# facebookresearch/metamorph

Measured on NVIDIA H100. Metric: interleaved tokens/sec (train step) LLaMA-3-8B+SigLIP seq4096, higher is better.
Workload: dtype bf16

## Files before the change

### metamorph_b200/csrc/gemm_tcgen05.cu

```cuda
#include "wgmma.cuh"
#include <mutex>
#include <stdlib.h>

namespace {

constexpr int BM = 128;
constexpr int BK = 64;
constexpr int kThreads = 384;
constexpr int kStageLd = 68;

enum Epilogue : int {
  EPI_STORE = 0,
  EPI_BIAS = 1,
  EPI_BIAS_GELU_ERF = 2,
  EPI_BIAS_GELU_TANH = 3,
  EPI_RESID = 4,
  EPI_BIAS_RESID = 5,
  EPI_SWIGLU = 6,
  EPI_SWIGLU_BWD = 7,
};

struct EpiParams {
  void* C;
  long long ldc;
  const bf16* bias;
  const bf16* resid;
  long long ldr;
  bf16* aux;
  long long ld_aux;
  int epi;
  int out_f32;
  int accumulate;
  float alpha;
};

template <int BN>
struct Cfg {
  static constexpr int kStages = (BN == 256) ? 3 : 5;
  static constexpr int kABytes = BM * BK * 2;
  static constexpr int kBBytes = BN * BK * 2;
  static constexpr int kStageBytes = kABytes + kBBytes;
  static constexpr int kEpiBytes = 2 * 64 * kStageLd * 4;
  static constexpr int kSmemBytes = kStages * kStageBytes + kEpiBytes + 1024  + 256 ;
  static_assert(kSmemBytes <= 227 * 1024, "shared memory budget of one H100 CTA");
};

__device__ __forceinline__ void epilogue_chunk(const EpiParams& ep, float (&v)[32], int row, bool row_ok,
                                               int col0, int N) {
    const bool full_chunk = (col0 + 32 <= N);

    if (ep.epi == EPI_SWIGLU_BWD) {
      if (row_ok) {
        bf16* gp = ep.aux + (long long)row * ep.ld_aux + 2 * col0;
        bf16* cp = reinterpret_cast<bf16*>(ep.C) + (long long)row * ep.ldc + col0;
#pragma unroll
        for (int blk = 0; blk < 2; ++blk) {
          uint32_t og[8], ou[8], oa[8];
#pragma unroll
          for (int hv = 0; hv < 2; ++hv) {
            const int4 graw = *reinterpret_cast<const int4*>(gp + blk * 32 + hv * 8);
            const int4 uraw = *reinterpret_cast<const int4*>(gp + blk * 32 + 16 + hv * 8);
            const uint32_t ug[4] = {(uint32_t)graw.x, (uint32_t)graw.y, (uint32_t)graw.z, (uint32_t)graw.w};
            const uint32_t uu[4] = {(uint32_t)uraw.x, (uint32_t)uraw.y, (uint32_t)uraw.z, (uint32_t)uraw.w};
#pragma unroll
            for (int j = 0; j < 4; ++j) {
              const float2 g = unpack_bf16x2(ug[j]);
              const float2 u = unpack_bf16x2(uu[j]);
              const float d0 = v[blk * 16 + hv * 8 + 2 * j], d1 = v[blk * 16 + hv * 8 + 2 * j + 1];
              const float s0 = 1.f / (1.f + __expf(-g.x)), s1 = 1.f / (1.f + __expf(-g.y));
              const float a0 = g.x * s0, a1 = g.y * s1;
// ... 102 lines not shown
            f = unpack_bf16x2(old.y); v[j + 2] += f.x; v[j + 3] += f.y;
            f = unpack_bf16x2(old.z); v[j + 4] += f.x; v[j + 5] += f.y;
            f = unpack_bf16x2(old.w); v[j + 6] += f.x; v[j + 7] += f.y;
          }
          int4 o;
          o.x = pack_bf16x2(v[j], v[j + 1]);
          o.y = pack_bf16x2(v[j + 2], v[j + 3]);
          o.z = pack_bf16x2(v[j + 4], v[j + 5]);
          o.w = pack_bf16x2(v[j + 6], v[j + 7]);
          *reinterpret_cast<int4*>(cp + j) = o;
        }
      } else {
        for (int j = 0; j < 32; ++j)
          if (col0 + j < N) {
            float x = v[j];
            if (ep.accumulate) x += __bfloat162float(cp[j]);
            cp[j] = __float2bfloat16(x);
          }
      }
    }
}

template <int BN, int TA, int TB>
__device__ __forceinline__ void wgmma_k16(float (&d)[BN / 2], uint64_t da, uint64_t db, uint32_t acc) {
  if constexpr (BN == 256) wgmma_m64n256_ss<TA, TB>(d, da, db, acc);
  else wgmma_m64n128_ss<TA, TB>(d, da, db, acc);
}

template <int BN, bool A_MN, bool B_MN>
__global__ void __launch_bounds__(kThreads, 1)
gemm_wgmma_kernel(const __grid_constant__ CUtensorMap tmap_a, const __grid_constant__ CUtensorMap tmap_b, int M, int N,
                  int K, int group_m, EpiParams ep) {
  using C = Cfg<BN>;
  extern __shared__ uint8_t smem_raw[];
  const uint32_t smem_base = (smem_u32(smem_raw) + 1023u) & ~1023u;
  const uint32_t epi_base = smem_base + C::kStages * C::kStageBytes;
  const uint32_t bar_base = epi_base + C::kEpiBytes;
  auto full_bar = [&](int s) { return bar_base + 8u * s; };
  auto empty_bar = [&](int s) { return bar_base + 8u * (C::kStages + s); };

  const int wg = threadIdx.x >> 7, lane = threadIdx.x & 31;
  const int num_m = (M + BM - 1) / BM, num_n = (N + BN - 1) / BN;
  const int num_tiles = num_m * num_n;
  const int num_kb = (K + BK - 1) / BK;

  if (threadIdx.x == 0) {
    prefetch_tmap(&tmap_a);
    prefetch_tmap(&tmap_b);
    for (int s = 0; s < C::kStages; ++s) {
      mbar_init(full_bar(s), 1);
      mbar_init(empty_bar(s), 8);
    }
    fence_barrier_init();
  }
  __syncthreads();

  auto tile_coords = [&](int t, int& m_blk, int& n_blk) {
    const int per_group = group_m * num_n;
    const int g = t / per_group;
    const int first_m = g * group_m;
    const int gsz = min(group_m, num_m - first_m);
    const int r = t - g * per_group;
    m_blk = first_m + (r % gsz);
    n_blk = r / gsz;
  };

  if (wg == 0) {
    setmaxnreg_dec<40>();
    if (threadIdx.x == 0) {
      int s = 0;
      uint32_t phase = 0;
      for (int t = blockIdx.x; t < num_tiles; t += gridDim.x) {
        int m_blk, n_blk;
        tile_coords(t, m_blk, n_blk);
        const int m0 = m_blk * BM, n0 = n_blk * BN;
        for (int kb = 0; kb < num_kb; ++kb) {
          mbar_wait(empty_bar(s), phase ^ 1);
          const uint32_t sa = smem_base + s * C::kStageBytes;
          const uint32_t sb = sa + C::kABytes;
          mbar_arrive_expect_tx(full_bar(s), C::kStageBytes);
          const int k0 = kb * BK;
          if constexpr (!A_MN) {
            tma_load_2d(sa, &tmap_a, full_bar(s), k0, m0);
          } else {
#pragma unroll
            for (int j = 0; j < BM / 64; ++j) tma_load_2d(sa + j * (BK * 128), &tmap_a, full_bar(s), m0 + 64 * j, k0);
          }
          if constexpr (!B_MN) {
            tma_load_2d(sb, &tmap_b, full_bar(s), k0, n0);
          } else {
#pragma unroll
            for (int j = 0; j < BN / 64; ++j) tma_load_2d(sb + j * (BK * 128), &tmap_b, full_bar(s), n0 + 64 * j, k0);
          }
          if (++s == C::kStages) { s = 0; phase ^= 1; }
        }
      }
    }
  } else {
    setmaxnreg_inc<232>();
    const int c = wg - 1;
    const int tid = threadIdx.x & 127, warp_in_wg = tid >> 5;
    constexpr uint32_t a_kstep = A_MN ? (16 * 128) : 32, b_kstep = B_MN ? (16 * 128) : 32;
    constexpr uint32_t a_lbo = A_MN ? (BK * 128) : 16, b_lbo = B_MN ? (BK * 128) : 16;
    float* stage = reinterpret_cast<float*>(smem_raw + (epi_base - smem_u32(smem_raw))) + c * 64 * kStageLd;
    const int er = tid & 63, ehalf = tid >> 6;
    int s = 0;
    uint32_t phase = 0;
    float d[BN / 2];
    for (int t = blockIdx.x; t < num_tiles; t += gridDim.x) {
      int m_blk, n_blk;
      tile_coords(t, m_blk, n_blk);
      for (int kb = 0; kb < num_kb; ++kb) {
        mbar_wait(full_bar(s), phase);
        const uint32_t sa = smem_base + s * C::kStageBytes + c * (64 * 128);
        const uint32_t sb = smem_base + s * C::kStageBytes + C::kABytes;
        wgmma_fence();
#pragma unroll
        for (int k = 0; k < BK / 16; ++k)
          wgmma_k16<BN, A_MN, B_MN>(d, wgmma_desc(sa + k * a_kstep, a_lbo), wgmma_desc(sb + k * b_kstep, b_lbo),
                                    (kb | k) != 0 ? 1u : 0u);
        wgmma_commit();
        wgmma_wait<0>();
        __syncwarp();
        if (lane == 0) mbar_arrive(empty_bar(s));
        if (++s == C::kStages) { s = 0; phase ^= 1; }
      }
      const int row = m_blk * BM + c * 64 + er;
      const bool row_ok = row < M;
      const int g = warp_in_wg * 16 + (lane >> 2), q2 = (lane & 3) * 2;
#pragma unroll
      for (int cc = 0; cc < BN / 64; ++cc) {
        const int colc = n_blk * BN + cc * 64;
        if (colc >= N) break;
        asm volatile("bar.sync %0, 128;" ::"r"(1 + c) : "memory");
#pragma unroll
        for (int j = 0; j < 8; ++j) {
          const float* src = d + 4 * (cc * 8 + j);
          *reinterpret_cast<float2*>(stage + g * kStageLd + j * 8 + q2) = make_float2(src[0], src[1]);
          *reinterpret_cast<float2*>(stage + (g + 8) * kStageLd + j * 8 + q2) = make_float2(src[2], src[3]);
        }
        asm volatile("bar.sync %0, 128;" ::"r"(1 + c) : "memory");
        const int col0 = colc + ehalf * 32;
        if (col0 < N) {
          float v[32];
          const float* rp = stage + er * kStageLd + ehalf * 32;
#pragma unroll
          for (int j = 0; j < 32; j += 4) {
            const float4 x = *reinterpret_cast<const float4*>(rp + j);
            v[j] = x.x * ep.alpha; v[j + 1] = x.y * ep.alpha; v[j + 2] = x.z * ep.alpha; v[j + 3] = x.w * ep.alpha;
          }
          epilogue_chunk(ep, v, row, row_ok, col0, N);
        }
      }
    }
  }
}

typedef CUresult (*PFN_encodeTiled)(CUtensorMap*, CUtensorMapDataType, cuuint32_t, void*,
                                    const cuuint64_t*, const cuuint64_t*, const cuuint32_t*,
                                    const cuuint32_t*, CUtensorMapInterleave, CUtensorMapSwizzle,
                                    CUtensorMapL2promotion, CUtensorMapFloatOOBfill);

PFN_encodeTiled get_encode_fn() {
  static PFN_encodeTiled fn = nullptr;
  static std::once_flag once;
  std::call_once(once, [] {
    void* p = nullptr;
    cudaDriverEntryPointQueryResult qres;
    if (cudaGetDriverEntryPoint("cuTensorMapEncodeTiled", &p, cudaEnableDefault, &qres) ==
            cudaSuccess &&
        qres == cudaDriverEntryPointSuccess)
      fn = reinterpret_cast<PFN_encodeTiled>(p);
  });
  return fn;
}

int make_tmap(CUtensorMap* tm, const void* base, long long inner, long long outer, long long ld,
              int box_inner, int box_outer) {
  PFN_encodeTiled enc = get_encode_fn();
  if (!enc) {
    mm_set_error("cuTensorMapEncodeTiled entry point unavailable (no CUDA driver?)");
    return MM_ERR_CUDA;
  }
  cuuint64_t dims[2] = {(cuuint64_t)inner, (cuuint64_t)outer};
// ... 112 lines not shown
```

### metamorph_b200/csrc/attention_bwd_tc.cu

```cuda
#include "attention_tc.cuh"

using namespace mm_attn_tc;

namespace {

constexpr int BW_THREADS = 384;
constexpr int BW_TILE = 32768;
constexpr int BW_SMEM = 6 * BW_TILE + 2048  + 256  + 1024 ;

struct BwdTcParams {
  const float* lse;
  float* lse2;
  float* delta;
  bf16* dq;
  bf16* dk;
  bf16* dv;
  const int* seqlens;
  const int* seg_start;
  const int2* work_q;
  const int2* work_k;
  long long lddq, lddk, lddv;
  int B, T, Tp, Hq, Hkv;
  float scale;
};

__device__ __forceinline__ void store_acc_rows(bf16* dst0, bf16* dst1, bool w0, bool w1, bool ok0, bool ok1,
                                               const float (&a)[64], int q2) {
#pragma unroll
  for (int t = 0; t < 16; ++t) {
    if (w0) *reinterpret_cast<uint32_t*>(dst0 + 8 * t + q2) = ok0 ? pack_bf16x2(a[4 * t], a[4 * t + 1]) : 0u;
    if (w1) *reinterpret_cast<uint32_t*>(dst1 + 8 * t + q2) = ok1 ? pack_bf16x2(a[4 * t + 2], a[4 * t + 3]) : 0u;
  }
}

__global__ void __launch_bounds__(BW_THREADS, 1)
flash_bwd_dq_kernel(const __grid_constant__ CUtensorMap tmap_q, const __grid_constant__ CUtensorMap tmap_k,
                    const __grid_constant__ CUtensorMap tmap_v, const __grid_constant__ CUtensorMap tmap_do,
                    const __grid_constant__ CUtensorMap tmap_o, BwdTcParams p) {
  extern __shared__ uint8_t smem_raw[];
// ... 108 lines not shown
  }
  const int g = ((threadIdx.x & 127) >> 5) * 16 + (lane >> 2), q2 = (lane & 3) * 2;
  int q_idx[2];
  bool q_ok[2];
  float delta[2], lse2[2];
#pragma unroll
  for (int i = 0; i < 2; ++i) {
    const int r = c * 64 + g + 8 * i;
    q_idx[i] = q0 + r;
    q_ok[i] = q_idx[i] < kv_len;
    delta[i] = q_ok[i] ? (sRed[r] + sRed[128 + r]) * p.scale : 0.f;
    lse2[i] = q_ok[i] ? p.lse[((long long)b * p.Hq + h) * p.T + q_idx[i]] * kLog2e : 0.f;
  }
  const float sl2 = p.scale * kLog2e;
  const uint32_t sQc = sQ + (uint32_t)c * 8192u, sdOc = sdO + (uint32_t)c * 8192u;
  float dq[64];
  for (int j = 0; j < n_tiles; ++j) {
    const int bf = j & 1;
    const uint32_t ph = (uint32_t)((j >> 1) & 1);
    mbar_wait(bf ? k_full1 : k_full0, ph);
    mbar_wait(bf ? v_full1 : v_full0, ph);
#pragma unroll 1
    for (int hf = 0; hf < 2; ++hf) {
      float s[32], dp[32];
      wgmma_fence();
#pragma unroll
      for (int k = 0; k < 8; ++k) {
        wgmma_m64n64_ss<0, 0>(s, desc_kmajor(sQc, k), desc_kmajor(sK[bf] + hf * 8192u, k), k != 0 ? 1u : 0u);
        wgmma_m64n64_ss<0, 0>(dp, desc_kmajor(sdOc, k), desc_kmajor(sV[bf] + hf * 8192u, k), k != 0 ? 1u : 0u);
      }
      wgmma_commit();
      wgmma_wait<0>();
      const int k0 = j * 128 + hf * 64;
#pragma unroll
      for (int t = 0; t < 32; ++t) {
        const int i = (t >> 1) & 1;
        const int col = k0 + (t >> 2) * 8 + q2 + (t & 1);
        const bool ok = q_ok[i] && col <= q_idx[i] && col < kv_len;
        const float pv = ok ? fast_exp2(fmaf(s[t], sl2, -lse2[i])) : 0.f;
        s[t] = pv * fmaf(dp[t], p.scale, -delta[i]);
      }
      uint32_t da[4][4];
#pragma unroll
      for (int k = 0; k < 4; ++k) acc_to_a(s, k, da[k]);
      wgmma_fence();
#pragma unroll
      for (int k = 0; k < 4; ++k)
        wgmma_m64n128_rs<1>(dq, da[k], desc_mnmajor(sK[bf], hf * 4 + k), (j | hf | k) != 0 ? 1u : 0u);
      wgmma_commit();
      wgmma_wait<0>();
    }
    consumer_release(bf ? k_empty1 : k_empty0);
    consumer_release(bf ? v_empty1 : v_empty0);
  }
  bf16* d0 = p.dq + (long long)(tok0 + q_idx[0]) * p.lddq + (long long)h * 128;
  bf16* d1 = p.dq + (long long)(tok0 + q_idx[1]) * p.lddq + (long long)h * 128;
  store_acc_rows(d0, d1, q_idx[0] < row_limit, q_idx[1] < row_limit, q_ok[0], q_ok[1], dq, q2);
}

__global__ void __launch_bounds__(BW_THREADS, 1)
flash_bwd_dkv_kernel(const __grid_constant__ CUtensorMap tmap_q, const __grid_constant__ CUtensorMap tmap_k,
                     const __grid_constant__ CUtensorMap tmap_v, const __grid_constant__ CUtensorMap tmap_do,
                     const __grid_constant__ CUtensorMap tmap_stat, BwdTcParams p) {
  extern __shared__ uint8_t smem_raw[];
  const int wg = threadIdx.x >> 7, lane = threadIdx.x & 31;
  const int jt = p.work_k ? 2 * p.work_k[blockIdx.x >> 1].y + (int)(blockIdx.x & 1) : (int)blockIdx.y;
  const int hk = p.work_k ? (int)blockIdx.y : (int)(blockIdx.x % p.Hkv);
  const int b = p.work_k ? p.work_k[blockIdx.x >> 1].x : (int)(blockIdx.x / p.Hkv);
  const int G = p.Hq / p.Hkv;
  const int kv0 = jt * 64;
  const int kv_len = p.seqlens ? min(p.seqlens[b], p.T) : p.T;
  const int tok0 = p.seg_start ? p.seg_start[b] : b * p.T;
  const int row_limit = p.seg_start ? kv_len : p.T;

  if (kv0 >= kv_len) {
    for (int i = threadIdx.x; i < 64 * 16; i += BW_THREADS) {
      const int r = i >> 4, c = (i & 15) * 8;
      if (kv0 + r < row_limit) {
        *reinterpret_cast<int4*>(p.dk + (long long)(tok0 + kv0 + r) * p.lddk + (long long)hk * 128 + c) = make_int4(0, 0, 0, 0);
        *reinterpret_cast<int4*>(p.dv + (long long)(tok0 + kv0 + r) * p.lddv + (long long)hk * 128 + c) = make_int4(0, 0, 0, 0);
      }
    }
    return;
  }
  const int qt_begin = kv0 / 128;
  const int n_qt = (kv_len + 127) / 128 - qt_begin;
  const int n_it = n_qt * G;

  const uint32_t base = (smem_u32(smem_raw) + 1023u) & ~1023u;
  uint8_t* base_ptr = smem_raw + (base - smem_u32(smem_raw));
  const uint32_t sK = base, sV = base + BW_TILE;
  const uint32_t sQ[2] = {base + 2 * BW_TILE, base + 4 * BW_TILE};
  const uint32_t sdO[2] = {base + 3 * BW_TILE, base + 5 * BW_TILE};
  const float* sStat = reinterpret_cast<const float*>(base_ptr + 6 * BW_TILE);
  const uint32_t uStat = base + 6 * BW_TILE;
  const uint32_t bar = base + 6 * BW_TILE + 2048;
  const uint32_t kv_full = bar, qdo_full0 = bar + 8, qdo_full1 = bar + 16, qdo_empty0 = bar + 24, qdo_empty1 = bar + 32;

  if (threadIdx.x == 0) {
    prefetch_tmap(&tmap_q);
    prefetch_tmap(&tmap_k);
    prefetch_tmap(&tmap_v);
    prefetch_tmap(&tmap_do);
    prefetch_tmap(&tmap_stat);
    mbar_init(kv_full, 1);
    mbar_init(qdo_full0, 1);
    mbar_init(qdo_full1, 1);
    mbar_init(qdo_empty0, 8);
    mbar_init(qdo_empty1, 8);
    fence_barrier_init();
  }
  __syncthreads();

  if (wg == 0) {
    setmaxnreg_dec<40>();
    if (threadIdx.x == 0) {
      mbar_arrive_expect_tx(kv_full, 4 * 64 * 128);
      tma_load_2d(sK, &tmap_k, kv_full, hk * 128, tok0 + kv0);
      tma_load_2d(sK + 16384, &tmap_k, kv_full, hk * 128 + 64, tok0 + kv0);
      tma_load_2d(sV, &tmap_v, kv_full, hk * 128, tok0 + kv0);
      tma_load_2d(sV + 16384, &tmap_v, kv_full, hk * 128 + 64, tok0 + kv0);
      for (int it = 0; it < n_it; ++it) {
        const int buf = it & 1, use = it >> 1;
        const int hq = hk * G + it / n_qt;
        const int q0 = (qt_begin + it % n_qt) * 128;
        const uint32_t full = buf ? qdo_full1 : qdo_full0, empty = buf ? qdo_empty1 : qdo_empty0;
        mbar_wait(empty, (uint32_t)((use & 1) ^ 1));
        mbar_arrive_expect_tx(full, 2 * BW_TILE + 1024);
        tma_load_2d(sQ[buf], &tmap_q, full, hq * 128, tok0 + q0);
        tma_load_2d(sQ[buf] + 16384, &tmap_q, full, hq * 128 + 64, tok0 + q0);
        tma_load_2d(sdO[buf], &tmap_do, full, hq * 128, tok0 + q0);
        tma_load_2d(sdO[buf] + 16384, &tmap_do, full, hq * 128 + 64, tok0 + q0);
        tma_load_2d(uStat + buf * 1024, &tmap_stat, full, q0, b * p.Hq + hq);
        tma_load_2d(uStat + buf * 1024 + 512, &tmap_stat, full, q0, (p.B + b) * p.Hq + hq);
      }
    }
    return;
  }

  setmaxnreg_inc<232>();
  const bool is_dk = wg == 2;
  const int g = ((threadIdx.x & 127) >> 5) * 16 + (lane >> 2), q2 = (lane & 3) * 2;
  int key_idx[2];
  bool key_ok[2];
#pragma unroll
  for (int i = 0; i < 2; ++i) {
    key_idx[i] = kv0 + g + 8 * i;
    key_ok[i] = key_idx[i] < kv_len;
  }
  const float sl2 = p.scale * kLog2e;
  float acc[64];
  mbar_wait(kv_full, 0);
  for (int it = 0; it < n_it; ++it) {
    const int buf = it & 1;
    const int q0 = (qt_begin + it % n_qt) * 128;
    mbar_wait(buf ? qdo_full1 : qdo_full0, (uint32_t)((it >> 1) & 1));
    const float* sLse = sStat + buf * 256;
    const float* sDelta = sLse + 128;
#pragma unroll 1
    for (int hf = 0; hf < 2; ++hf) {
      float s[32], dp[32];
      uint32_t fa[4][4];
      wgmma_fence();
#pragma unroll
      for (int k = 0; k < 8; ++k) {
        wgmma_m64n64_ss<0, 0>(s, desc_kmajor(sK, k), desc_kmajor(sQ[buf] + hf * 8192u, k), k != 0 ? 1u : 0u);
        wgmma_m64n64_ss<0, 0>(dp, desc_kmajor(sV, k), desc_kmajor(sdO[buf] + hf * 8192u, k), k != 0 ? 1u : 0u);
      }
      wgmma_commit();
      wgmma_wait<0>();
#pragma unroll
      for (int t = 0; t < 32; ++t) {
        const int i = (t >> 1) & 1;
        const int ql = hf * 64 + (t >> 2) * 8 + q2 + (t & 1);
        const bool ok = key_ok[i] && (q0 + ql < kv_len) && (key_idx[i] <= q0 + ql);
        const float pv = ok ? fast_exp2(fmaf(s[t], sl2, -sLse[ql])) : 0.f;
        s[t] = is_dk ? pv * fmaf(dp[t], p.scale, -sDelta[ql]) : pv;
      }
#pragma unroll
      for (int k = 0; k < 4; ++k) acc_to_a(s, k, fa[k]);
      const uint32_t sB = is_dk ? sQ[buf] : sdO[buf];
      wgmma_fence();
#pragma unroll
      for (int k = 0; k < 4; ++k)
        wgmma_m64n128_rs<1>(acc, fa[k], desc_mnmajor(sB, hf * 4 + k), (it | hf | k) != 0 ? 1u : 0u);
      wgmma_commit();
      wgmma_wait<0>();
    }
    consumer_release(buf ? qdo_empty1 : qdo_empty0);
  }
  bf16* dst = is_dk ? p.dk : p.dv;
  const long long ld = is_dk ? p.lddk : p.lddv;
  store_acc_rows(dst + (long long)(tok0 + key_idx[0]) * ld + (long long)hk * 128,
                 dst + (long long)(tok0 + key_idx[1]) * ld + (long long)hk * 128, key_idx[0] < row_limit,
                 key_idx[1] < row_limit, key_ok[0], key_ok[1], acc, q2);
}

}

MM_API long long mm_attn_bwd_tc_workspace_bytes(int B, int T, int Hq) {
  const long long Tp = ((long long)T + 127) / 128 * 128;
  return 2 * (((long long)B * Hq * Tp * 4 + 255) / 256 * 256);
}

namespace {

int launch_bwd_tc(const void* q, const void* k, const void* v, const void* o, const void* dout, const float* lse, void* dq,
                  void* dk, void* dv, const int* seqlens, const int* seg_start, const int* work_q, int n_work_q,
                  const int* work_k, int n_work_k, long long total_rows, long long ldq, long long ldk, long long ldv,
                  long long ldo, long long lddo, long long lddq, long long lddk, long long lddv, int B, int T, int Hq,
                  int Hkv, float scale, void* workspace, long long workspace_bytes, cudaStream_t stream) {
  MM_CHECK_ARG(B > 0 && T > 0 && Hq > 0 && Hkv > 0 && Hq % Hkv == 0, "mm_attn_bwd_tc: bad shape");
  MM_CHECK_ARG(workspace != nullptr && workspace_bytes >= mm_attn_bwd_tc_workspace_bytes(B, T, Hq),
               "mm_attn_bwd_tc: workspace too small (use mm_attn_bwd_tc_workspace_bytes)");
  MM_CHECK_ARG(ldq % 8 == 0 && ldk % 8 == 0 && ldv % 8 == 0 && ldo % 8 == 0 && lddo % 8 == 0 && lddq % 8 == 0 &&
                   lddk % 8 == 0 && lddv % 8 == 0, "mm_attn_bwd_tc: pitches %% 8");
  MM_CHECK_ARG(((uintptr_t)q & 15) == 0 && ((uintptr_t)k & 15) == 0 && ((uintptr_t)v & 15) == 0 &&
                   ((uintptr_t)o & 15) == 0 && ((uintptr_t)dout & 15) == 0 && ((uintptr_t)dq & 15) == 0 &&
                   ((uintptr_t)dk & 15) == 0 && ((uintptr_t)dv & 15) == 0 && ((uintptr_t)workspace & 15) == 0,
               "mm_attn_bwd_tc: 16-byte alignment required");
  const int Tp = (T + 127) / 128 * 128;
  const long long stat_bytes = ((long long)B * Hq * Tp * 4 + 255) / 256 * 256;
  CUtensorMap tq, tk, tv, tdo, to, tstat, tk64, tv64;
  int rc;
  MM_CHECK_ARG(stat_bytes == (long long)B * Hq * Tp * 4, "mm_attn_bwd_tc: statistics rows must be contiguous");
  if ((rc = mm_attn_make_tmap_stats(&tstat, reinterpret_cast<const float*>(workspace), Tp, 2LL * B * Hq))) return rc;
  if ((rc = mm_attn_make_tmap_rows(&tq, q, (long long)Hq * 128, total_rows, ldq))) return rc;
  if ((rc = mm_attn_make_tmap_rows(&tk, k, (long long)Hkv * 128, total_rows, ldk))) return rc;
  if ((rc = mm_attn_make_tmap_rows(&tv, v, (long long)Hkv * 128, total_rows, ldv))) return rc;
  if ((rc = mm_attn_make_tmap_rows(&tdo, dout, (long long)Hq * 128, total_rows, lddo))) return rc;
  if ((rc = mm_attn_make_tmap_rows(&to, o, (long long)Hq * 128, total_rows, ldo))) return rc;
  if ((rc = mm_attn_make_tmap_rows(&tk64, k, (long long)Hkv * 128, total_rows, ldk, 64))) return rc;
  if ((rc = mm_attn_make_tmap_rows(&tv64, v, (long long)Hkv * 128, total_rows, ldv, 64))) return rc;
  static std::once_flag once;
  static cudaError_t err = cudaSuccess;
  std::call_once(once, [&] {
    err = cudaFuncSetAttribute(flash_bwd_dq_kernel, cudaFuncAttributeMaxDynamicSharedMemorySize, BW_SMEM);
    if (err == cudaSuccess)
      err = cudaFuncSetAttribute(flash_bwd_dkv_kernel, cudaFuncAttributeMaxDynamicSharedMemorySize, BW_SMEM);
  });
  MM_CHECK_CUDA(err);
  BwdTcParams p;
  p.lse = lse;
  p.lse2 = reinterpret_cast<float*>(workspace);
  p.delta = reinterpret_cast<float*>(reinterpret_cast<uint8_t*>(workspace) + stat_bytes);
  p.dq = (bf16*)dq; p.dk = (bf16*)dk; p.dv = (bf16*)dv; p.seqlens = seqlens; p.seg_start = seg_start;
  p.work_q = reinterpret_cast<const int2*>(work_q); p.work_k = reinterpret_cast<const int2*>(work_k);
  p.lddq = lddq; p.lddk = lddk; p.lddv = lddv;
  p.B = B; p.T = T; p.Tp = Tp; p.Hq = Hq; p.Hkv = Hkv; p.scale = scale;
  const int n_tiles = (T + 127) / 128;
  const dim3 grid_q = work_q ? dim3(n_work_q, Hq, 1) : dim3(n_tiles, Hq, B);
  const dim3 grid_k = work_k ? dim3(2 * n_work_k, Hkv, 1) : dim3(Hkv * B, 2 * n_tiles, 1);
  flash_bwd_dq_kernel<<<grid_q, BW_THREADS, BW_SMEM, stream>>>(tq, tk, tv, tdo, to, p);
  MM_CHECK_LAUNCH();
  flash_bwd_dkv_kernel<<<grid_k, BW_THREADS, BW_SMEM, stream>>>(tq, tk64, tv64, tdo, tstat, p);
  MM_CHECK_LAUNCH();
  return MM_OK;
}

}

MM_API int mm_attn_bwd_tc(const void* q, const void* k, const void* v, const void* o, const void* dout,
                          const float* lse, void* dq, void* dk, void* dv, const int* seqlens, long long ldq,
                          long long ldk, long long ldv, long long ldo, long long lddo, long long lddq,
                          long long lddk, long long lddv, int B, int T, int Hq, int Hkv, int head_dim,
                          float scale, void* workspace, long long workspace_bytes, cudaStream_t stream) {
  MM_CHECK_ARG(head_dim == 128, "mm_attn_bwd_tc: head_dim must be 128");
  return launch_bwd_tc(q, k, v, o, dout, lse, dq, dk, dv, seqlens, nullptr, nullptr, 0, nullptr, 0, (long long)B * T, ldq,
                       ldk, ldv, ldo, lddo, lddq, lddk, lddv, B, T, Hq, Hkv, scale, workspace, workspace_bytes, stream);
}

MM_API int mm_attn_bwd_tc_varlen(const void* q, const void* k, const void* v, const void* o, const void* dout,
                                 const float* lse, void* dq, void* dk, void* dv, const int* seg_start,
                                 const int* seg_len, int n_seg, int max_len, const int* work_q, int n_work_q,
                                 const int* work_k, int n_work_k, long long total_rows, long long ldq, long long ldk,
                                 long long ldv, long long ldo, long long lddo, long long lddq, long long lddk,
                                 long long lddv, int Hq, int Hkv, int head_dim, float scale, void* workspace,
                                 long long workspace_bytes, cudaStream_t stream) {
  MM_CHECK_ARG(head_dim == 128, "mm_attn_bwd_tc_varlen: head_dim must be 128");
  MM_CHECK_ARG(seg_start != nullptr && seg_len != nullptr && work_q != nullptr && work_k != nullptr && n_work_q > 0 &&
                   n_work_k > 0 && n_seg > 0 && max_len > 0, "mm_attn_bwd_tc_varlen: segment tables missing");
  return launch_bwd_tc(q, k, v, o, dout, lse, dq, dk, dv, seg_len, seg_start, work_q, n_work_q, work_k, n_work_k,
                       total_rows, ldq, ldk, ldv, ldo, lddo, lddq, lddk, lddv, n_seg, max_len, Hq, Hkv, scale, workspace,
                       workspace_bytes, stream);
}
```

### metamorph_b200/csrc/attention_tc.cu

```cuda
#include "attention_tc.cuh"

using namespace mm_attn_tc;

namespace {

constexpr int TC_BR = 128, TC_BC = 128, TC_D = 128;
constexpr int TC_TILE_BYTES = 128 * 128 * 2;

struct TcFwdParams {
  bf16* o;
  float* lse;
  const int* seqlens;
  const int* seg_start;
  const int2* work;
  long long ldo;
  int B, T, Hq, Hkv;
  float scale;
  int causal;
};

constexpr int TC_THREADS = 384;
constexpr int TC_SMEM = 5 * TC_TILE_BYTES + 256 + 1024;

__global__ void __launch_bounds__(TC_THREADS, 1)
// ... 153 lines not shown
}

static PFN_encodeTiled tmap_encoder() {
  static PFN_encodeTiled enc = nullptr;
  static std::once_flag once;
  std::call_once(once, [] {
    void* fn = nullptr;
    cudaDriverEntryPointQueryResult q;
    if (cudaGetDriverEntryPoint("cuTensorMapEncodeTiled", &fn, cudaEnableDefault, &q) == cudaSuccess &&
        q == cudaDriverEntryPointSuccess)
      enc = reinterpret_cast<PFN_encodeTiled>(fn);
  });
  if (!enc) mm_set_error("cuTensorMapEncodeTiled unavailable");
  return enc;
}

int mm_attn_make_tmap_stats(CUtensorMap* tm, const float* base, long long width, long long rows) {
  PFN_encodeTiled enc = tmap_encoder();
  if (!enc) return MM_ERR_CUDA;
  cuuint64_t dims[2] = {(cuuint64_t)width, (cuuint64_t)rows};
  cuuint64_t strides[1] = {(cuuint64_t)width * 4};
  cuuint32_t box[2] = {128, 1};
  cuuint32_t estr[2] = {1, 1};
  CUresult r = enc(tm, CU_TENSOR_MAP_DATA_TYPE_FLOAT32, 2, const_cast<float*>(base), dims, strides, box, estr,
                   CU_TENSOR_MAP_INTERLEAVE_NONE, CU_TENSOR_MAP_SWIZZLE_NONE, CU_TENSOR_MAP_L2_PROMOTION_NONE,
                   CU_TENSOR_MAP_FLOAT_OOB_FILL_NONE);
  if (r != CUDA_SUCCESS) {
    mm_set_error("cuTensorMapEncodeTiled failed (%d) for the attention statistics rows", (int)r);
    return MM_ERR_CUDA;
  }
  return MM_OK;
}

int mm_attn_make_tmap_rows(CUtensorMap* tm, const void* base, long long width, long long rows, long long ld,
                           int box_rows) {
  PFN_encodeTiled enc = tmap_encoder();
  if (!enc) return MM_ERR_CUDA;
  cuuint64_t dims[2] = {(cuuint64_t)width, (cuuint64_t)rows};
  cuuint64_t strides[1] = {(cuuint64_t)ld * 2};
  cuuint32_t box[2] = {64, (cuuint32_t)box_rows};
  cuuint32_t estr[2] = {1, 1};
  CUresult r = enc(tm, CU_TENSOR_MAP_DATA_TYPE_BFLOAT16, 2, const_cast<void*>(base), dims, strides, box, estr,
                   CU_TENSOR_MAP_INTERLEAVE_NONE, CU_TENSOR_MAP_SWIZZLE_128B, CU_TENSOR_MAP_L2_PROMOTION_L2_256B,
                   CU_TENSOR_MAP_FLOAT_OOB_FILL_NONE);
  if (r != CUDA_SUCCESS) {
    mm_set_error("cuTensorMapEncodeTiled failed (%d) for attention operand", (int)r);
    return MM_ERR_CUDA;
  }
  return MM_OK;
}


namespace {

int launch_fwd_tc(const void* q, const void* k, const void* v, void* o, float* lse, const int* seqlens,
                  const int* seg_start, const int* work, int n_work, long long total_rows, long long ldq, long long ldk,
                  long long ldv, long long ldo, int B, int T, int Hq, int Hkv, int causal, float scale,
                  cudaStream_t stream) {
  MM_CHECK_ARG(B > 0 && T > 0 && Hq > 0 && Hkv > 0 && Hq % Hkv == 0, "mm_attn_fwd_tc: bad head counts");
  MM_CHECK_ARG(ldq % 8 == 0 && ldk % 8 == 0 && ldv % 8 == 0 && ldo % 8 == 0 &&
                   ((uintptr_t)q & 15) == 0 && ((uintptr_t)k & 15) == 0 && ((uintptr_t)v & 15) == 0 &&
                   ((uintptr_t)o & 15) == 0, "mm_attn_fwd_tc: 16-byte alignment / pitch %% 8 required");
  CUtensorMap tq, tk, tv;
  int rc;
  if ((rc = mm_attn_make_tmap_rows(&tq, q, (long long)Hq * 128, total_rows, ldq))) return rc;
  if ((rc = mm_attn_make_tmap_rows(&tk, k, (long long)Hkv * 128, total_rows, ldk))) return rc;
  if ((rc = mm_attn_make_tmap_rows(&tv, v, (long long)Hkv * 128, total_rows, ldv))) return rc;
  TcFwdParams p;
  p.o = (bf16*)o; p.lse = lse; p.seqlens = seqlens; p.seg_start = seg_start;
  p.work = reinterpret_cast<const int2*>(work); p.ldo = ldo;
  p.B = B; p.T = T; p.Hq = Hq; p.Hkv = Hkv; p.scale = scale; p.causal = causal;
  const dim3 grid = work ? dim3(n_work, Hq, 1) : dim3((T + TC_BR - 1) / TC_BR, Hq, B);
  static std::once_flag once;
// ... 32 lines not shown
```

### metamorph_b200/csrc/attention_tc.cuh

```cuda
#pragma once
#include "wgmma.cuh"
#include <mutex>

namespace mm_attn_tc {

constexpr float kLog2e = 1.4426950408889634f;

__device__ __forceinline__ float fast_exp2(float x) {
  float y;
  asm("ex2.approx.ftz.f32 %0, %1;" : "=f"(y) : "f"(x));
  return y;
}

__device__ __forceinline__ uint64_t desc_kmajor(uint32_t tile, int k16) {
  return wgmma_desc(tile + (uint32_t)(k16 >> 2) * 16384u + (uint32_t)(k16 & 3) * 32u, 16);
}
__device__ __forceinline__ uint64_t desc_mnmajor(uint32_t tile, int k16) {
  return wgmma_desc(tile + (uint32_t)k16 * 2048u, 16384);
}
template <int NA>
__device__ __forceinline__ void acc_to_a(const float (&d)[NA], int k, uint32_t (&a)[4]) {
#pragma unroll
  for (int i = 0; i < 4; ++i) a[i] = pack_bf16x2(d[8 * k + 2 * i], d[8 * k + 2 * i + 1]);
}
__device__ __forceinline__ void consumer_release(uint32_t bar) {
  __syncwarp();
  if ((threadIdx.x & 31) == 0) mbar_arrive(bar);
}

}

int mm_attn_make_tmap_rows(CUtensorMap* tm, const void* base, long long width, long long rows, long long ld,
                           int box_rows = 128);
int mm_attn_make_tmap_stats(CUtensorMap* tm, const float* base, long long width, long long rows);
```

Baseline: 34660.

## Add ping-pong consumer warpgroup schedule for BN=128 GEMM tiles

For BN=128, each consumer warpgroup now owns a whole 128-row tile, and the two warpgroups alternate tiles. Named barriers order their mainloops so one group's epilogue overlaps the other's MMA. The mainloop also keeps one wgmma batch in flight (wait<1>) and releases the previous stage late, instead of waiting fully every k-block. This targets tensor-core idle time during epilogues, at the cost of double the accumulator registers and more barrier coordination.

Result: no change. 34860 (median of 6 runs) (+0.6%).

```diff
diff --git a/metamorph_b200/csrc/gemm_tcgen05.cu b/metamorph_b200/csrc/gemm_tcgen05.cu
--- a/metamorph_b200/csrc/gemm_tcgen05.cu
+++ b/metamorph_b200/csrc/gemm_tcgen05.cu
@@ -34,8 +34,18 @@
   float alpha;
 };
 
+constexpr int kOrderBar = 3;
+
+__device__ __forceinline__ void named_bar_sync(int id, int n) {
+  asm volatile("bar.sync %0, %1;" ::"r"(id), "r"(n) : "memory");
+}
+__device__ __forceinline__ void named_bar_arrive(int id, int n) {
+  asm volatile("bar.arrive %0, %1;" ::"r"(id), "r"(n) : "memory");
+}
+
 template <int BN>
 struct Cfg {
+  static constexpr bool kPingPong = (BN == 128);
   static constexpr int kStages = (BN == 256) ? 3 : 5;
   static constexpr int kABytes = BM * BK * 2;
   static constexpr int kBBytes = BN * BK * 2;
@@ -204,6 +214,8 @@
 gemm_wgmma_kernel(const __grid_constant__ CUtensorMap tmap_a, const __grid_constant__ CUtensorMap tmap_b, int M, int N,
                   int K, int group_m, EpiParams ep) {
   using C = Cfg<BN>;
+  constexpr bool kPingPong = C::kPingPong;
+  constexpr int kBlocks = kPingPong ? 2 : 1;
   extern __shared__ uint8_t smem_raw[];
   const uint32_t smem_base = (smem_u32(smem_raw) + 1023u) & ~1023u;
   const uint32_t epi_base = smem_base + C::kStages * C::kStageBytes;
@@ -221,7 +233,7 @@
     prefetch_tmap(&tmap_b);
     for (int s = 0; s < C::kStages; ++s) {
       mbar_init(full_bar(s), 1);
-      mbar_init(empty_bar(s), 8);
+      mbar_init(empty_bar(s), kPingPong ? 4 : 8);
     }
     fence_barrier_init();
   }
@@ -274,54 +286,76 @@
     const int tid = threadIdx.x & 127, warp_in_wg = tid >> 5;
     constexpr uint32_t a_kstep = A_MN ? (16 * 128) : 32, b_kstep = B_MN ? (16 * 128) : 32;
     constexpr uint32_t a_lbo = A_MN ? (BK * 128) : 16, b_lbo = B_MN ? (BK * 128) : 16;
+    const uint32_t a_off = kPingPong ? 0u : (uint32_t)c * (64 * 128);
     float* stage = reinterpret_cast<float*>(smem_raw + (epi_base - smem_u32(smem_raw))) + c * 64 * kStageLd;
     const int er = tid & 63, ehalf = tid >> 6;
+    auto release = [&](int st) {
+      __syncwarp();
+      if (lane == 0) mbar_arrive(empty_bar(st));
+    };
     int s = 0;
     uint32_t phase = 0;
-    float d[BN / 2];
-    for (int t = blockIdx.x; t < num_tiles; t += gridDim.x) {
+    float d[kBlocks][BN / 2];
+    int i = 0;
+    for (int t = blockIdx.x; t < num_tiles; t += gridDim.x, ++i) {
+      if (kPingPong && (i & 1) != c) {
+        const int adv = s + num_kb;
+        s = adv % C::kStages;
+        phase ^= (uint32_t)(adv / C::kStages) & 1u;
+        continue;
+      }
       int m_blk, n_blk;
       tile_coords(t, m_blk, n_blk);
+      if (kPingPong && i > 0) named_bar_sync(kOrderBar + c, 256);
+      int s_prev = 0;
       for (int kb = 0; kb < num_kb; ++kb) {
         mbar_wait(full_bar(s), phase);
-        const uint32_t sa = smem_base + s * C::kStageBytes + c * (64 * 128);
+        const uint32_t sa = smem_base + s * C::kStageBytes + a_off;
         const uint32_t sb = smem_base + s * C::kStageBytes + C::kABytes;
         wgmma_fence();
 #pragma unroll
         for (int k = 0; k < BK / 16; ++k)
-          wgmma_k16<BN, A_MN, B_MN>(d, wgmma_desc(sa + k * a_kstep, a_lbo), wgmma_desc(sb + k * b_kstep, b_lbo),
-                                    (kb | k) != 0 ? 1u : 0u);
+#pragma unroll
+          for (int h = 0; h < kBlocks; ++h)
+            wgmma_k16<BN, A_MN, B_MN>(d[h], wgmma_desc(sa + h * (64 * 128) + k * a_kstep, a_lbo),
+                                      wgmma_desc(sb + k * b_kstep, b_lbo), (kb | k) != 0 ? 1u : 0u);
         wgmma_commit();
-        wgmma_wait<0>();
-        __syncwarp();
-        if (lane == 0) mbar_arrive(empty_bar(s));
+        wgmma_wait<1>();
+        if (kb > 0) release(s_prev);
+        s_prev = s;
         if (++s == C::kStages) { s = 0; phase ^= 1; }
       }
-      const int row = m_blk * BM + c * 64 + er;
-      const bool row_ok = row < M;
+      if (kPingPong && t + (int)gridDim.x < num_tiles) named_bar_arrive(kOrderBar + (c ^ 1), 256);
+      wgmma_wait<0>();
+      release(s_prev);
       const int g = warp_in_wg * 16 + (lane >> 2), q2 = (lane & 3) * 2;
 #pragma unroll
-      for (int cc = 0; cc < BN / 64; ++cc) {
-        const int colc = n_blk * BN + cc * 64;
-        if (colc >= N) break;
-        asm volatile("bar.sync %0, 128;" ::"r"(1 + c) : "memory");
-#pragma unroll
-        for (int j = 0; j < 8; ++j) {
-          const float* src = d + 4 * (cc * 8 + j);
-          *reinterpret_cast<float2*>(stage + g * kStageLd + j * 8 + q2) = make_float2(src[0], src[1]);
-          *reinterpret_cast<float2*>(stage + (g + 8) * kStageLd + j * 8 + q2) = make_float2(src[2], src[3]);
-        }
-        asm volatile("bar.sync %0, 128;" ::"r"(1 + c) : "memory");
-        const int col0 = colc + ehalf * 32;
-        if (col0 < N) {
-          float v[32];
-          const float* rp = stage + er * kStageLd + ehalf * 32;
-#pragma unroll
-          for (int j = 0; j < 32; j += 4) {
-            const float4 x = *reinterpret_cast<const float4*>(rp + j);
-            v[j] = x.x * ep.alpha; v[j + 1] = x.y * ep.alpha; v[j + 2] = x.z * ep.alpha; v[j + 3] = x.w * ep.alpha;
-          }
-          epilogue_chunk(ep, v, row, row_ok, col0, N);
+      for (int h = 0; h < kBlocks; ++h) {
+        const int row = m_blk * BM + (kPingPong ? h : c) * 64 + er;
+        const bool row_ok = row < M;
+#pragma unroll
+        for (int cc = 0; cc < BN / 64; ++cc) {
+          const int colc = n_blk * BN + cc * 64;
+          if (colc >= N) break;
+          named_bar_sync(1 + c, 128);
+#pragma unroll
+          for (int j = 0; j < 8; ++j) {
+            const float* src = d[h] + 4 * (cc * 8 + j);
+            *reinterpret_cast<float2*>(stage + g * kStageLd + j * 8 + q2) = make_float2(src[0], src[1]);
+            *reinterpret_cast<float2*>(stage + (g + 8) * kStageLd + j * 8 + q2) = make_float2(src[2], src[3]);
+          }
+          named_bar_sync(1 + c, 128);
+          const int col0 = colc + ehalf * 32;
+          if (col0 < N) {
+            float v[32];
+            const float* rp = stage + er * kStageLd + ehalf * 32;
+#pragma unroll
+            for (int j = 0; j < 32; j += 4) {
+              const float4 x = *reinterpret_cast<const float4*>(rp + j);
+              v[j] = x.x * ep.alpha; v[j + 1] = x.y * ep.alpha; v[j + 2] = x.z * ep.alpha; v[j + 3] = x.w * ep.alpha;
+            }
+            epilogue_chunk(ep, v, row, row_ok, col0, N);
+          }
         }
       }
     }
```

## Compute dK and dV together per warpgroup over 128-row KV tiles; skip unneeded masking

Applied to the files above, without the earlier changes.

The dK/dV backward kernel now uses 256 threads with no dedicated producer warpgroup. Each of the two consumer warpgroups owns 64 of 128 KV rows and accumulates both dK and dV, instead of one warpgroup doing dK and the other dV over 64 rows. Thread 0 issues the TMA prefetches inline, and the 64-row K/V tensor maps are dropped. Both the dQ and dK/dV kernels gain an unmasked fast path for tiles fully inside the causal and length bounds, which avoids per-element predicate work. The trade-offs are higher register pressure from holding two accumulators and the loss of warp-specialized producer overlap.

Result: faster. 25260 before, 25730 after (median of 6 runs) (+1.9%).

```diff
diff --git a/metamorph_b200/csrc/attention_bwd_tc.cu b/metamorph_b200/csrc/attention_bwd_tc.cu
--- a/metamorph_b200/csrc/attention_bwd_tc.cu
+++ b/metamorph_b200/csrc/attention_bwd_tc.cu
@@ -5,6 +5,7 @@
 namespace {
 
 constexpr int BW_THREADS = 384;
+constexpr int DKV_THREADS = 256;
 constexpr int BW_TILE = 32768;
 constexpr int BW_SMEM = 6 * BW_TILE + 2048  + 256  + 1024 ;
 
@@ -179,13 +180,21 @@
       wgmma_commit();
       wgmma_wait<0>();
       const int k0 = j * 128 + hf * 64;
-#pragma unroll
-      for (int t = 0; t < 32; ++t) {
-        const int i = (t >> 1) & 1;
-        const int col = k0 + (t >> 2) * 8 + q2 + (t & 1);
-        const bool ok = q_ok[i] && col <= q_idx[i] && col < kv_len;
-        const float pv = ok ? fast_exp2(fmaf(s[t], sl2, -lse2[i])) : 0.f;
-        s[t] = pv * fmaf(dp[t], p.scale, -delta[i]);
+      if (k0 + 64 > q0 || k0 + 64 > kv_len || q0 + 128 > kv_len) {
+#pragma unroll
+        for (int t = 0; t < 32; ++t) {
+          const int i = (t >> 1) & 1;
+          const int col = k0 + (t >> 2) * 8 + q2 + (t & 1);
+          const bool ok = q_ok[i] && col <= q_idx[i] && col < kv_len;
+          const float pv = ok ? fast_exp2(fmaf(s[t], sl2, -lse2[i])) : 0.f;
+          s[t] = pv * fmaf(dp[t], p.scale, -delta[i]);
+        }
+      } else {
+#pragma unroll
+        for (int t = 0; t < 32; ++t) {
+          const int i = (t >> 1) & 1;
+          s[t] = fast_exp2(fmaf(s[t], sl2, -lse2[i])) * fmaf(dp[t], p.scale, -delta[i]);
+        }
       }
       uint32_t da[4][4];
 #pragma unroll
@@ -205,27 +214,27 @@
   store_acc_rows(d0, d1, q_idx[0] < row_limit, q_idx[1] < row_limit, q_ok[0], q_ok[1], dq, q2);
 }
 
-__global__ void __launch_bounds__(BW_THREADS, 1)
+__global__ void __launch_bounds__(DKV_THREADS, 1)
 flash_bwd_dkv_kernel(const __grid_constant__ CUtensorMap tmap_q, const __grid_constant__ CUtensorMap tmap_k,
                      const __grid_constant__ CUtensorMap tmap_v, const __grid_constant__ CUtensorMap tmap_do,
                      const __grid_constant__ CUtensorMap tmap_stat, BwdTcParams p) {
   extern __shared__ uint8_t smem_raw[];
-  const int wg = threadIdx.x >> 7, lane = threadIdx.x & 31;
-  const int jt = p.work_k ? 2 * p.work_k[blockIdx.x >> 1].y + (int)(blockIdx.x & 1) : (int)blockIdx.y;
+  const int c = threadIdx.x >> 7, lane = threadIdx.x & 31;
+  const int jt = p.work_k ? p.work_k[blockIdx.x].y : (int)blockIdx.y;
   const int hk = p.work_k ? (int)blockIdx.y : (int)(blockIdx.x % p.Hkv);
-  const int b = p.work_k ? p.work_k[blockIdx.x >> 1].x : (int)(blockIdx.x / p.Hkv);
+  const int b = p.work_k ? p.work_k[blockIdx.x].x : (int)(blockIdx.x / p.Hkv);
   const int G = p.Hq / p.Hkv;
-  const int kv0 = jt * 64;
+  const int kv0 = jt * 128;
   const int kv_len = p.seqlens ? min(p.seqlens[b], p.T) : p.T;
   const int tok0 = p.seg_start ? p.seg_start[b] : b * p.T;
   const int row_limit = p.seg_start ? kv_len : p.T;
 
   if (kv0 >= kv_len) {
-    for (int i = threadIdx.x; i < 64 * 16; i += BW_THREADS) {
-      const int r = i >> 4, c = (i & 15) * 8;
+    for (int i = threadIdx.x; i < 128 * 16; i += DKV_THREADS) {
+      const int r = i >> 4, col = (i & 15) * 8;
       if (kv0 + r < row_limit) {
-        *reinterpret_cast<int4*>(p.dk + (long long)(tok0 + kv0 + r) * p.lddk + (long long)hk * 128 + c) = make_int4(0, 0, 0, 0);
-        *reinterpret_cast<int4*>(p.dv + (long long)(tok0 + kv0 + r) * p.lddv + (long long)hk * 128 + c) = make_int4(0, 0, 0, 0);
+        *reinterpret_cast<int4*>(p.dk + (long long)(tok0 + kv0 + r) * p.lddk + (long long)hk * 128 + col) = make_int4(0, 0, 0, 0);
+        *reinterpret_cast<int4*>(p.dv + (long long)(tok0 + kv0 + r) * p.lddv + (long long)hk * 128 + col) = make_int4(0, 0, 0, 0);
       }
     }
     return;
@@ -259,44 +268,40 @@
   }
   __syncthreads();
 
-  if (wg == 0) {
-    setmaxnreg_dec<40>();
-    if (threadIdx.x == 0) {
-      mbar_arrive_expect_tx(kv_full, 4 * 64 * 128);
-      tma_load_2d(sK, &tmap_k, kv_full, hk * 128, tok0 + kv0);
-      tma_load_2d(sK + 16384, &tmap_k, kv_full, hk * 128 + 64, tok0 + kv0);
-      tma_load_2d(sV, &tmap_v, kv_full, hk * 128, tok0 + kv0);
-      tma_load_2d(sV + 16384, &tmap_v, kv_full, hk * 128 + 64, tok0 + kv0);
-      for (int it = 0; it < n_it; ++it) {
-        const int buf = it & 1, use = it >> 1;
-        const int hq = hk * G + it / n_qt;
-        const int q0 = (qt_begin + it % n_qt) * 128;
-        const uint32_t full = buf ? qdo_full1 : qdo_full0, empty = buf ? qdo_empty1 : qdo_empty0;
-        mbar_wait(empty, (uint32_t)((use & 1) ^ 1));
-        mbar_arrive_expect_tx(full, 2 * BW_TILE + 1024);
-        tma_load_2d(sQ[buf], &tmap_q, full, hq * 128, tok0 + q0);
-        tma_load_2d(sQ[buf] + 16384, &tmap_q, full, hq * 128 + 64, tok0 + q0);
-        tma_load_2d(sdO[buf], &tmap_do, full, hq * 128, tok0 + q0);
-        tma_load_2d(sdO[buf] + 16384, &tmap_do, full, hq * 128 + 64, tok0 + q0);
-        tma_load_2d(uStat + buf * 1024, &tmap_stat, full, q0, b * p.Hq + hq);
-        tma_load_2d(uStat + buf * 1024 + 512, &tmap_stat, full, q0, (p.B + b) * p.Hq + hq);
-      }
-    }
-    return;
-  }
-
-  setmaxnreg_inc<232>();
-  const bool is_dk = wg == 2;
+  auto load_qdo = [&](int it) {
+    const int buf = it & 1;
+    const int hq = hk * G + it / n_qt;
+    const int q0 = (qt_begin + it % n_qt) * 128;
+    const uint32_t full = buf ? qdo_full1 : qdo_full0;
+    mbar_arrive_expect_tx(full, 2 * BW_TILE + 1024);
+    tma_load_2d(sQ[buf], &tmap_q, full, hq * 128, tok0 + q0);
+    tma_load_2d(sQ[buf] + 16384, &tmap_q, full, hq * 128 + 64, tok0 + q0);
+    tma_load_2d(sdO[buf], &tmap_do, full, hq * 128, tok0 + q0);
+    tma_load_2d(sdO[buf] + 16384, &tmap_do, full, hq * 128 + 64, tok0 + q0);
+    tma_load_2d(uStat + buf * 1024, &tmap_stat, full, q0, b * p.Hq + hq);
+    tma_load_2d(uStat + buf * 1024 + 512, &tmap_stat, full, q0, (p.B + b) * p.Hq + hq);
+  };
+  if (threadIdx.x == 0) {
+    mbar_arrive_expect_tx(kv_full, 2 * BW_TILE);
+    tma_load_2d(sK, &tmap_k, kv_full, hk * 128, tok0 + kv0);
+    tma_load_2d(sK + 16384, &tmap_k, kv_full, hk * 128 + 64, tok0 + kv0);
+    tma_load_2d(sV, &tmap_v, kv_full, hk * 128, tok0 + kv0);
+    tma_load_2d(sV + 16384, &tmap_v, kv_full, hk * 128 + 64, tok0 + kv0);
+    load_qdo(0);
+    if (n_it > 1) load_qdo(1);
+  }
+
   const int g = ((threadIdx.x & 127) >> 5) * 16 + (lane >> 2), q2 = (lane & 3) * 2;
   int key_idx[2];
   bool key_ok[2];
 #pragma unroll
   for (int i = 0; i < 2; ++i) {
-    key_idx[i] = kv0 + g + 8 * i;
+    key_idx[i] = kv0 + c * 64 + g + 8 * i;
     key_ok[i] = key_idx[i] < kv_len;
   }
   const float sl2 = p.scale * kLog2e;
-  float acc[64];
+  const uint32_t sKc = sK + (uint32_t)c * 8192u, sVc = sV + (uint32_t)c * 8192u;
+  float dv[64], dk[64];
   mbar_wait(kv_full, 0);
   for (int it = 0; it < n_it; ++it) {
     const int buf = it & 1;
@@ -304,43 +309,66 @@
     mbar_wait(buf ? qdo_full1 : qdo_full0, (uint32_t)((it >> 1) & 1));
     const float* sLse = sStat + buf * 256;
     const float* sDelta = sLse + 128;
+    const bool need_mask = q0 == kv0 || q0 + 128 > kv_len || kv0 + 128 > kv_len;
 #pragma unroll 1
     for (int hf = 0; hf < 2; ++hf) {
       float s[32], dp[32];
-      uint32_t fa[4][4];
       wgmma_fence();
 #pragma unroll
       for (int k = 0; k < 8; ++k) {
-        wgmma_m64n64_ss<0, 0>(s, desc_kmajor(sK, k), desc_kmajor(sQ[buf] + hf * 8192u, k), k != 0 ? 1u : 0u);
-        wgmma_m64n64_ss<0, 0>(dp, desc_kmajor(sV, k), desc_kmajor(sdO[buf] + hf * 8192u, k), k != 0 ? 1u : 0u);
+        wgmma_m64n64_ss<0, 0>(s, desc_kmajor(sKc, k), desc_kmajor(sQ[buf] + hf * 8192u, k), k != 0 ? 1u : 0u);
+        wgmma_m64n64_ss<0, 0>(dp, desc_kmajor(sVc, k), desc_kmajor(sdO[buf] + hf * 8192u, k), k != 0 ? 1u : 0u);
       }
       wgmma_commit();
       wgmma_wait<0>();
-#pragma unroll
-      for (int t = 0; t < 32; ++t) {
-        const int i = (t >> 1) & 1;
-        const int ql = hf * 64 + (t >> 2) * 8 + q2 + (t & 1);
-        const bool ok = key_ok[i] && (q0 + ql < kv_len) && (key_idx[i] <= q0 + ql);
-        const float pv = ok ? fast_exp2(fmaf(s[t], sl2, -sLse[ql])) : 0.f;
-        s[t] = is_dk ? pv * fmaf(dp[t], p.scale, -sDelta[ql]) : pv;
-      }
-#pragma unroll
-      for (int k = 0; k < 4; ++k) acc_to_a(s, k, fa[k]);
-      const uint32_t sB = is_dk ? sQ[buf] : sdO[buf];
+      if (need_mask) {
+#pragma unroll
+        for (int t = 0; t < 32; ++t) {
+          const int i = (t >> 1) & 1;
+          const int ql = hf * 64 + (t >> 2) * 8 + q2 + (t & 1);
+          const bool ok = key_ok[i] && (q0 + ql < kv_len) && (key_idx[i] <= q0 + ql);
+          const float pv = ok ? fast_exp2(fmaf(s[t], sl2, -sLse[ql])) : 0.f;
+          s[t] = pv;
+          dp[t] = pv * fmaf(dp[t], p.scale, -sDelta[ql]);
+        }
+      } else {
+#pragma unroll
+        for (int t = 0; t < 32; ++t) {
+          const int ql = hf * 64 + (t >> 2) * 8 + q2 + (t & 1);
+          const float pv = fast_exp2(fmaf(s[t], sl2, -sLse[ql]));
+          s[t] = pv;
+          dp[t] = pv * fmaf(dp[t], p.scale, -sDelta[ql]);
+        }
+      }
+      uint32_t pa[4][4], dsa[4][4];
+#pragma unroll
+      for (int k = 0; k < 4; ++k) {
+        acc_to_a(s, k, pa[k]);
+        acc_to_a(dp, k, dsa[k]);
+      }
       wgmma_fence();
 #pragma unroll
       for (int k = 0; k < 4; ++k)
-        wgmma_m64n128_rs<1>(acc, fa[k], desc_mnmajor(sB, hf * 4 + k), (it | hf | k) != 0 ? 1u : 0u);
+        wgmma_m64n128_rs<1>(dv, pa[k], desc_mnmajor(sdO[buf], hf * 4 + k), (it | hf | k) != 0 ? 1u : 0u);
+#pragma unroll
+      for (int k = 0; k < 4; ++k)
+        wgmma_m64n128_rs<1>(dk, dsa[k], desc_mnmajor(sQ[buf], hf * 4 + k), (it | hf | k) != 0 ? 1u : 0u);
       wgmma_commit();
       wgmma_wait<0>();
     }
     consumer_release(buf ? qdo_empty1 : qdo_empty0);
-  }
-  bf16* dst = is_dk ? p.dk : p.dv;
-  const long long ld = is_dk ? p.lddk : p.lddv;
-  store_acc_rows(dst + (long long)(tok0 + key_idx[0]) * ld + (long long)hk * 128,
-                 dst + (long long)(tok0 + key_idx[1]) * ld + (long long)hk * 128, key_idx[0] < row_limit,
-                 key_idx[1] < row_limit, key_ok[0], key_ok[1], acc, q2);
+    if (threadIdx.x == 0 && it + 2 < n_it) {
+      mbar_wait(buf ? qdo_empty1 : qdo_empty0, (uint32_t)((it >> 1) & 1));
+      load_qdo(it + 2);
+    }
+    __syncwarp();
+  }
+  const long long r0 = tok0 + key_idx[0], r1 = tok0 + key_idx[1];
+  const bool w0 = key_idx[0] < row_limit, w1 = key_idx[1] < row_limit;
+  store_acc_rows(p.dv + r0 * p.lddv + (long long)hk * 128, p.dv + r1 * p.lddv + (long long)hk * 128, w0, w1, key_ok[0],
+                 key_ok[1], dv, q2);
+  store_acc_rows(p.dk + r0 * p.lddk + (long long)hk * 128, p.dk + r1 * p.lddk + (long long)hk * 128, w0, w1, key_ok[0],
+                 key_ok[1], dk, q2);
 }
 
 }
@@ -368,7 +396,7 @@
                "mm_attn_bwd_tc: 16-byte alignment required");
   const int Tp = (T + 127) / 128 * 128;
   const long long stat_bytes = ((long long)B * Hq * Tp * 4 + 255) / 256 * 256;
-  CUtensorMap tq, tk, tv, tdo, to, tstat, tk64, tv64;
+  CUtensorMap tq, tk, tv, tdo, to, tstat;
   int rc;
   MM_CHECK_ARG(stat_bytes == (long long)B * Hq * Tp * 4, "mm_attn_bwd_tc: statistics rows must be contiguous");
   if ((rc = mm_attn_make_tmap_stats(&tstat, reinterpret_cast<const float*>(workspace), Tp, 2LL * B * Hq))) return rc;
@@ -377,8 +405,6 @@
   if ((rc = mm_attn_make_tmap_rows(&tv, v, (long long)Hkv * 128, total_rows, ldv))) return rc;
   if ((rc = mm_attn_make_tmap_rows(&tdo, dout, (long long)Hq * 128, total_rows, lddo))) return rc;
   if ((rc = mm_attn_make_tmap_rows(&to, o, (long long)Hq * 128, total_rows, ldo))) return rc;
-  if ((rc = mm_attn_make_tmap_rows(&tk64, k, (long long)Hkv * 128, total_rows, ldk, 64))) return rc;
-  if ((rc = mm_attn_make_tmap_rows(&tv64, v, (long long)Hkv * 128, total_rows, ldv, 64))) return rc;
   static std::once_flag once;
   static cudaError_t err = cudaSuccess;
   std::call_once(once, [&] {
@@ -397,10 +423,10 @@
   p.B = B; p.T = T; p.Tp = Tp; p.Hq = Hq; p.Hkv = Hkv; p.scale = scale;
   const int n_tiles = (T + 127) / 128;
   const dim3 grid_q = work_q ? dim3(n_work_q, Hq, 1) : dim3(n_tiles, Hq, B);
-  const dim3 grid_k = work_k ? dim3(2 * n_work_k, Hkv, 1) : dim3(Hkv * B, 2 * n_tiles, 1);
+  const dim3 grid_k = work_k ? dim3(n_work_k, Hkv, 1) : dim3(Hkv * B, n_tiles, 1);
   flash_bwd_dq_kernel<<<grid_q, BW_THREADS, BW_SMEM, stream>>>(tq, tk, tv, tdo, to, p);
   MM_CHECK_LAUNCH();
-  flash_bwd_dkv_kernel<<<grid_k, BW_THREADS, BW_SMEM, stream>>>(tq, tk64, tv64, tdo, tstat, p);
+  flash_bwd_dkv_kernel<<<grid_k, DKV_THREADS, BW_SMEM, stream>>>(tq, tk, tv, tdo, tstat, p);
   MM_CHECK_LAUNCH();
   return MM_OK;
 }
diff --git a/metamorph_b200/csrc/attention_tc.cu b/metamorph_b200/csrc/attention_tc.cu
--- a/metamorph_b200/csrc/attention_tc.cu
+++ b/metamorph_b200/csrc/attention_tc.cu
@@ -209,13 +209,12 @@
   return MM_OK;
 }
 
-int mm_attn_make_tmap_rows(CUtensorMap* tm, const void* base, long long width, long long rows, long long ld,
-                           int box_rows) {
+int mm_attn_make_tmap_rows(CUtensorMap* tm, const void* base, long long width, long long rows, long long ld) {
   PFN_encodeTiled enc = tmap_encoder();
   if (!enc) return MM_ERR_CUDA;
   cuuint64_t dims[2] = {(cuuint64_t)width, (cuuint64_t)rows};
   cuuint64_t strides[1] = {(cuuint64_t)ld * 2};
-  cuuint32_t box[2] = {64, (cuuint32_t)box_rows};
+  cuuint32_t box[2] = {64, 128};
   cuuint32_t estr[2] = {1, 1};
   CUresult r = enc(tm, CU_TENSOR_MAP_DATA_TYPE_BFLOAT16, 2, const_cast<void*>(base), dims, strides, box, estr,
                    CU_TENSOR_MAP_INTERLEAVE_NONE, CU_TENSOR_MAP_SWIZZLE_128B, CU_TENSOR_MAP_L2_PROMOTION_L2_256B,
diff --git a/metamorph_b200/csrc/attention_tc.cuh b/metamorph_b200/csrc/attention_tc.cuh
--- a/metamorph_b200/csrc/attention_tc.cuh
+++ b/metamorph_b200/csrc/attention_tc.cuh
@@ -30,6 +30,5 @@
 
 }
 
-int mm_attn_make_tmap_rows(CUtensorMap* tm, const void* base, long long width, long long rows, long long ld,
-                           int box_rows = 128);
+int mm_attn_make_tmap_rows(CUtensorMap* tm, const void* base, long long width, long long rows, long long ld);
 int mm_attn_make_tmap_stats(CUtensorMap* tm, const float* base, long long width, long long rows);
```
